# JianCao92/speaker-diarization

Hardware: AMD Instinct MI355X
Metric: diarized audio throughput (CD gw/BIC + CL hi/BIC) (higher is better)
Workload: dtype f64

## Files before the change

include/spkd.h:

```cpp
#ifndef SPKD_H
#define SPKD_H

#include <stddef.h>
#include <stdint.h>

#ifdef __cplusplus
extern "C" {
#endif

#define SPKD_ABI_VERSION 2
#define SPKD_DIM 39
#define SPKD_REC 820

typedef enum {
    SPKD_OK = 0,
    SPKD_EINVAL = 1,
    SPKD_EHIP = 2,
    SPKD_ENONFINITE = 3,
    SPKD_EOVERFLOW = 4,
    SPKD_ENOMEM = 5
} spkd_status;

typedef enum { SPKD_BIC = 0, SPKD_GLR = 1, SPKD_KL2 = 2, SPKD_KL2_PINV = 3 } spkd_kind;

// ... 103 lines not shown
    const int32_t *turn;
    const int64_t *frame_b;
    const int64_t *frame_e;
    const int64_t *index;
    const int64_t *d_index;
    const int64_t *redo_line;
    const int64_t *redo_begin;
    const int64_t *redo_end;
} spkd_gw_lines_view;

spkd_status spkd_gw_batch(spkd_ctx *ctx, const float *d_frames, int64_t n_frames,
                          const int64_t *h_turn_begin, const int64_t *h_turn_end, int64_t n_turns,
                          const spkd_cd_params *params, const int64_t *h_ev_off,
                          const double *h_turn_start_s, const double *h_turn_end_s,
                          const int64_t *h_turn_file_off, const int64_t *h_turn_file_len,
                          double *d_seg_stats, int want_index, spkd_gw_lines_view *view);

int64_t spkd_sw_window_count(int64_t turn_len, double winsize, double winstep);
spkd_status spkd_sw(spkd_ctx *ctx, const float *d_frames, int64_t n_frames,
                    const int64_t *h_turn_begin, const int64_t *h_turn_end, int64_t n_turns,
                    const spkd_cd_params *params, const int64_t *h_d_off, double *h_d);

enum { SPKD_AHC_AUTO = 0, SPKD_AHC_MONO = 1, SPKD_AHC_WIDE = 2 };

typedef struct {
    int32_t variant;
    int32_t kind;
    int32_t max_spk;
    int32_t path;
    double lambdac;
    double threshold;
} spkd_ahc_params;

spkd_status spkd_ahc(spkd_ctx *ctx, const double *d_stats, const int64_t *h_seg_off,
                     int64_t n_problems, const spkd_ahc_params *params,
                     int32_t *h_n_merges, int32_t *h_merge_a, int32_t *h_merge_b,
                     double *h_merge_d, double *h_stat_max, double *h_stat_min);

spkd_status spkd_ahc_matrix(spkd_ctx *ctx, const double *d_stats, int64_t n, const spkd_ahc_params *params,
                            const double *d_matrix, double stat_max_in, double stat_min_in,
                            int32_t *h_n_merges, int32_t *h_merge_a, int32_t *h_merge_b,
                            double *h_merge_d, double *h_stat_max, double *h_stat_min);

spkd_status spkd_ahc_fused(spkd_ctx *ctx, const float *d_frames, int64_t n_frames,
                           const double *d_records, int64_t n_records, int64_t *d_line_index,
                           const int64_t *h_seg_off, int64_t n_problems,
// ... 59 lines not shown
```

speaker-diarization_amd/csrc/spkd_cluster.hpp:

```cpp
#pragma once
#include "spkd_device.hpp"
#include "spkd_quad.hpp"
#include "spkd_tri.hpp"
#include "../../include/spkd.h"

namespace spkd {

constexpr double MAXINT_F = 9223372036854775808.0;
constexpr double PEN_UNIT = 39.0 + 0.5 * 39.0 * 40.0;
constexpr int AUX = 3 * DA;
constexpr int ERR_DEGENERATE_MERGE = 2;

__device__ __forceinline__ unsigned long long dkey(double v) {
    unsigned long long b = (unsigned long long)__double_as_longlong(v);
    return (b >> 63) ? ~b : (b | 0x8000000000000000ull);
}
__device__ __forceinline__ double dkey_inv(unsigned long long k) {
    unsigned long long b = (k >> 63) ? (k & 0x7fffffffffffffffull) : ~k;
    return __longlong_as_double((long long)b);
}
template <bool MAXOP>
__device__ __forceinline__ unsigned wave_red_u32(unsigned x) {
    auto op = [](unsigned a, unsigned b) { return MAXOP ? (a > b ? a : b) : (a < b ? a : b); };
    x = op(x, (unsigned)__builtin_amdgcn_update_dpp((int)x, (int)x, 0xB1, 0xf, 0xf, false));
// ... 476 lines not shown
            }
            if (valid && stat_valid(d)) {
                wmax = (wmax != wmax || d > wmax) ? d : wmax;
                wmin = (wmin != wmin || d < wmin) ? d : wmin;
            }
        }
    }
    if (variant == 1 && (kind == SPKD_KL2 ? lane_id() == 0 : L.t == 0)) {
        if (wmax == wmax) atomicMax(stat_max + p, dkey(wmax));
        if (wmin == wmin) atomicMin(stat_min + p, dkey(wmin));
    }
}

constexpr int AHC_WAVES = 8;
constexpr int AHC_TPB = AHC_WAVES * WAVE;

#ifdef SPKD_PROFILE
__device__ unsigned long long g_step_prof[8];
__device__ unsigned long long g_ahc_prof[8];
#endif
constexpr int NO_COL = 0x7fffffff;
constexpr int AHC_MAX_N = 65536;

__device__ __forceinline__ void refresh_rows(const double* __restrict__ Dm, long long N,
                                             const int32_t* __restrict__ al, int32_t* __restrict__ dirty,
                                             double* __restrict__ rmin, int32_t* __restrict__ rarg,
                                             int32_t* __restrict__ rnan, unsigned long long* masks,
                                             int tid, int wave, int lane) {
    const long long n_chunks = (N + WAVE - 1) / WAVE;
    for (long long ch = wave; ch < n_chunks; ch += AHC_WAVES) {
        const long long rl = ch * WAVE + lane;
        const long long rc = rl < N ? rl : N - 1;
        const int fa = al[rc], fd = dirty[rc];
        const unsigned long long mk = __ballot(rl < N && fa && fd);
        if (lane == 0) masks[ch] = mk;
    }
    __syncthreads();
    int ord = 0;
    for (long long ch = 0; ch < n_chunks; ++ch) {
        const long long r0 = ch * WAVE;
        unsigned long long todo = masks[ch];
        while (todo) {
            const int b = __builtin_ctzll(todo);
            todo &= todo - 1;
            if ((ord++ & (AHC_WAVES - 1)) != wave) continue;
            const long long r = r0 + b;
            const double* row = Dm + r * N;
            double mv = __builtin_huge_val();
            int mc = NO_COL, nc = NO_COL;
            for (long long c0 = 0; c0 < N; c0 += 4 * WAVE) {
                double v[4];
                int a[4];
#pragma unroll
                for (int u = 0; u < 4; ++u) {
                    const long long c = c0 + u * WAVE + lane;
                    const long long cc = c < N ? c : N - 1;
                    a[u] = (c < N) ? al[cc] : 0;
                    v[u] = row[cc];
                }
#pragma unroll
                for (int u = 0; u < 4; ++u) {
                    const int c = (int)(c0 + u * WAVE + lane);
                    if (!a[u]) continue;
                    if (v[u] != v[u]) { if (c < nc) nc = c; continue; }
                    if (v[u] < mv || (v[u] == mv && c < mc)) { mv = v[u]; mc = c; }
                }
            }
            {
                unsigned long long okey;
                unsigned oc;
                wave_argmin_key(mc != NO_COL ? dkey(mv) : ~0ull, (unsigned)mc, okey, oc);
                mv = okey != ~0ull ? dkey_inv(okey) : __builtin_huge_val();
                mc = okey != ~0ull ? (int)oc : NO_COL;
                nc = __any(nc != NO_COL) ? (int)wave_red_u32<false>((unsigned)nc) : NO_COL;
            }
            if (lane == 0) { rmin[r] = mv; rarg[r] = mc; rnan[r] = nc; dirty[r] = 0; }
#ifdef SPKD_PROFILE
            if (lane == 0) atomicAdd(&g_ahc_prof[0], 1ull);
#endif
        }
    }
}

template <bool TWO>
__global__ __launch_bounds__(AHC_TPB) void k_ahc(
        double* __restrict__ ex, double* __restrict__ pk, const int64_t* __restrict__ seg_off,
        int variant, int kind, int max_spk, double lambdac, double threshold,
        double* __restrict__ ld, double* __restrict__ aux,
        double* __restrict__ mat, const int64_t* __restrict__ mat_off,
        int32_t* __restrict__ alive, double* __restrict__ tmp,
        double* __restrict__ rmin_all, int32_t* __restrict__ rcache_all,
        int32_t* __restrict__ out_n, int32_t* __restrict__ out_a, int32_t* __restrict__ out_b,
        double* __restrict__ out_d, unsigned long long* stat_max, unsigned long long* stat_min,
        double* __restrict__ final_max, double* __restrict__ final_min, int* err,
        double* pinv_ws) {
    extern __shared__ int32_t ids[];
    __shared__ double ldsA[QREC];
    __shared__ unsigned long long red3[AHC_WAVES][3];
    __shared__ unsigned long long s_masks[AHC_MAX_N / WAVE];
    __shared__ int s_cnt[2];
    __shared__ int s_nids;
    __shared__ int s_next;
    __shared__ double s_tmax[AHC_WAVES];
    const int tid = threadIdx.x, lane = lane_id(), wave = tid >> 6;
    const QuadLane L = quad_lane();
    const int p = blockIdx.x;
    const int64_t off = seg_off[p];
    const long long N = seg_off[p + 1] - off;
    double* Dm = mat + mat_off[p];
    int32_t* al = alive + off;
    double* ldp = ld + off;
    double* tp = tmp + off;
    double* rmin = rmin_all + off;
    int32_t* rarg = rcache_all + 3 * off;
    int32_t* rnan = rarg + N;
    int32_t* dirty = rnan + N;
    for (long long c = tid; c < N; c += AHC_TPB) { al[c] = 1; dirty[c] = 1; }
    __syncthreads();
    long long m = N;
    int n_merges = 0;
    const long long INF_IDX = 0x7fffffffffffffffLL;
    double fmin = 0.0;
#ifdef SPKD_PROFILE
    unsigned long long ahc_acc[5] = {0ull, 0ull, 0ull, 0ull, 0ull}, ahc_t = clock64();
#define AHC_TICK(i) do { const unsigned long long now_ = clock64(); ahc_acc[i] += now_ - ahc_t; ahc_t = now_; } while (0)
#else
#define AHC_TICK(i) ((void)0)
#endif
    while (true) {
        refresh_rows(Dm, N, al, dirty, rmin, rarg, rnan, s_masks, tid, wave, lane);
        __syncthreads();
        AHC_TICK(0);
        unsigned long long kb = ~0ull, ib = ~0ull, inan = ~0ull;
        for (long long r = tid; r < N; r += AHC_TPB) {
            if (!al[r]) continue;
            const double v = rmin[r];
            const int c = rarg[r], nc = rnan[r];
            if (nc != NO_COL) { const unsigned long long l = (unsigned long long)(r * N + nc); inan = l < inan ? l : inan; }
            if (c != NO_COL) {
                const unsigned long long kv = dkey(v);
                if (kv < kb) { kb = kv; ib = (unsigned long long)(r * N + c); }
            }
        }
        {
            const unsigned long long wk = wave_red_u64<false>(kb);
            const unsigned long long wi = wave_red_u64<false>(kb == wk ? ib : ~0ull);
            const unsigned long long wn = __any(inan != ~0ull) ? wave_red_u64<false>(inan) : ~0ull;
            if (lane == 0) { red3[wave][0] = wk; red3[wave][1] = wi; red3[wave][2] = wn; }
        }
        __syncthreads();
        unsigned long long bk = red3[0][0], bi = red3[0][1], bn = red3[0][2];
#pragma unroll
        for (int w = 1; w < AHC_WAVES; ++w) {
            const unsigned long long ok = red3[w][0], oi = red3[w][1], on = red3[w][2];
            const bool t = ok < bk || (ok == bk && oi < bi);
            bk = t ? ok : bk; bi = t ? oi : bi;
            bn = on < bn ? on : bn;
        }
        const bool has_nan = bn != ~0ull;
        const double mind = has_nan ? __builtin_nan("") : (bi != ~0ull ? dkey_inv(bk) : __builtin_huge_val());
        const long long index = has_nan ? (long long)bn : (bi != ~0ull ? (long long)bi : INF_IDX);
        fmin = mind;
        const bool go = (mind <= threshold) || (max_spk > 0 && m > max_spk);
        if (!go) break;
        AHC_TICK(1);
        const long long r0 = index / N, c0 = index - r0 * N;
        if (r0 == c0) {
            if (tid == 0) atomicOr(err, ERR_DEGENERATE_MERGE);
            break;
        }
        const long long sa = r0 < c0 ? r0 : c0, sb = r0 < c0 ? c0 : r0;
        if (tid < 2) s_cnt[tid] = 0;
        if (tid == 0) { s_nids = 1; s_next = 0; }
        __syncthreads();
        {
            int ca = 0, cb = 0;
            for (long long c = tid; c < sb; c += AHC_TPB) {
                if (al[c]) { cb++; if (c < sa) ca++; }
            }
            ca = __builtin_amdgcn_readlane(wave_scan_i32(ca), WAVE - 1);
            cb = __builtin_amdgcn_readlane(wave_scan_i32(cb), WAVE - 1);
            if (lane == 0 && ca) atomicAdd(&s_cnt[0], ca);
            if (lane == 0 && cb) atomicAdd(&s_cnt[1], cb);
        }
        __syncthreads();
        if (tid == 0) {
            const int64_t o = off + n_merges;
            out_a[o] = s_cnt[0]; out_b[o] = s_cnt[1]; out_d[o] = mind;
            al[sb] = 0;
            ids[0] = (int32_t)sa;
        }
        n_merges++;
        m--;
#ifdef SPKD_PROFILE
        if (tid == 0) atomicAdd(&g_ahc_prof[1], 1ull);
#endif
        double* A = ex + (off + sa) * QREC;
        const double* B = ex + (off + sb) * QREC;
        {
            double* Ap = pk + (off + sa) * REC;
            const double* Bp = pk + (off + sb) * REC;
            constexpr int NQ = (QREC + AHC_TPB - 1) / AHC_TPB, NP = (REC + AHC_TPB - 1) / AHC_TPB;
            double qa[NQ], qb[NQ], pa[NP], pb[NP];
#pragma unroll
            for (int u = 0; u < NQ; ++u) {
                const int e = tid + u * AHC_TPB;
                qa[u] = A[e < QREC ? e : 0]; qb[u] = B[e < QREC ? e : 0];
            }
#pragma unroll
            for (int u = 0; u < NP; ++u) {
                const int e = tid + u * AHC_TPB;
                pa[u] = Ap[e < REC ? e : 0]; pb[u] = Bp[e < REC ? e : 0];
            }
#pragma unroll
            for (int u = 0; u < NQ; ++u) {
                const int e = tid + u * AHC_TPB;
                const double v = qa[u] + qb[u];
                if (e < QREC) { A[e] = v; ldsA[e] = v; }
            }
#pragma unroll
            for (int u = 0; u < NP; ++u) {
                const int e = tid + u * AHC_TPB;
                if (e < REC) Ap[e] = pa[u] + pb[u];
            }
        }
        __syncthreads();
        for (long long c0 = 0; c0 < N; c0 += AHC_TPB) {
            const long long c = c0 + tid;
            const bool take = c < N && c != sa && al[c < N ? c : N - 1];
            const unsigned long long mk = __ballot(take);
            int base = 0;
            if (lane == 0 && mk) base = atomicAdd(&s_nids, __popcll(mk));
            base = __shfl(base, 0);
            if (take) ids[base + __popcll(mk & ((1ull << lane) - 1ull))] = (int32_t)c;
        }
        __syncthreads();
        AHC_TICK(2);
        const int nids = s_nids;
        const double nA = ldsA[QREC_COUNT_AT];
        if (kind == SPKD_KL2) {
            if (wave == 0) {
                double a[DA];
                single_rows_from_qr(A, a);
                const double mean_i = a[D] / nA;
                cov_rows(a, nA);
                kl2_aux_from_cov(a, mean_i, aux + (off + sa) * AUX, pinv_ws);
            }
        } else {
            for (;;) {
                int q4 = 0;
                if (lane == 0) q4 = atomicAdd(&s_next, 1);
                const int base = 4 * __builtin_amdgcn_readfirstlane(q4);
                if (base >= nids) break;
                int k = base + L.m;
                const bool valid = k < nids;
                k = valid ? k : nids - 1;
                const int32_t slot = ids[k];
                const double v = quad_pair_det<TWO>(kind, ldsA, nA, A, ex + (off + slot) * QREC, pk + (off + slot) * REC, k == 0, L, err);
                if (valid && L.t == 0) {
                    if (k == 0) ldp[sa] = log(v); else tp[slot] = v;
                }
            }
        }
        __syncthreads();
        AHC_TICK(3);
        double wmax = __builtin_nan(""), wmin = __builtin_nan("");
        const double ldA = ldp[sa];
        for (long long c = tid; c < N; c += AHC_TPB) {
            if (c == sa || !al[c]) continue;
            double d;
            if (kind == SPKD_KL2) {
                const double* a1 = aux + (off + sa) * AUX;
                const double* a2 = aux + (off + c) * AUX;
                double t1 = 0.0, t2 = 0.0;
                for (int i = 0; i < D; ++i) {
                    const float dm = (float)a1[2 * DA + i] - (float)a2[2 * DA + i];
                    const double delta = (double)dm;
                    t1 += (a1[i] - a2[i]) * (a2[DA + i] - a1[DA + i]);
                    t2 += ((a1[DA + i] + a2[DA + i]) * delta) * delta;
                }
                d = 0.5 * t1 + 0.5 * t2;
            } else {
                const double nC = qr_count(ex + (off + c) * QREC);
                d = finish_distance(kind, lambdac, nA, ldA, nC, ldp[c], log(tp[c]));
            }
            Dm[sa * N + c] = d;
            const int ra = rarg[c], rn = rnan[c];
            if (variant == 1) {
                Dm[c * N + sa] = d;
                if (ra == sa || ra == sb || rn == sa || rn == sb) {
                    if (rn != sa && rn != sb && d < rmin[c]) { rmin[c] = d; rarg[c] = (int)sa; }
                    else dirty[c] = 1;
                }
                else if (d != d) { if ((int)sa < rn) rnan[c] = (int)sa; }
                else if (d < rmin[c] || (d == rmin[c] && (int)sa < ra)) { rmin[c] = d; rarg[c] = (int)sa; }
                if (stat_valid(d)) {
                    wmax = (wmax != wmax || d > wmax) ? d : wmax;
                    wmin = (wmin != wmin || d < wmin) ? d : wmin;
                }
            } else {
                if (ra == sb || rn == sb) dirty[c] = 1;
            }
        }
        if (tid == 0) dirty[sa] = 1;
        if (variant == 1) {
            const unsigned long long kmax = wave_red_u64<true>(wmax == wmax ? dkey(wmax) : 0ull);
            const unsigned long long kmin = wave_red_u64<false>(wmin == wmin ? dkey(wmin) : ~0ull);
            if (lane == 0) {
                if (kmax != 0ull) atomicMax(stat_max + p, kmax);
                if (kmin != ~0ull) atomicMin(stat_min + p, kmin);
            }
        }
        __syncthreads();
        AHC_TICK(4);
    }
#ifdef SPKD_PROFILE
    if (tid == 0) for (int i = 0; i < 5; ++i) atomicAdd(&g_ahc_prof[2 + i], ahc_acc[i]);
#endif
    double tmax = -__builtin_huge_val();
    bool anynan = false;
    for (long long r = wave; r < N; r += AHC_WAVES) {
        if (!al[r]) continue;
        const double* row = Dm + r * N;
        for (long long c = lane; c < N; c += WAVE) {
            if (!al[c]) continue;
            const double v = row[c];
            if (v != v) anynan = true; else tmax = v > tmax ? v : tmax;
        }
    }
#pragma unroll
    for (int s = 1; s < WAVE; s <<= 1) {
        const double t2 = __shfl_xor(tmax, s);
        tmax = t2 > tmax ? t2 : tmax;
    }
    anynan = __any(anynan);
    if (lane == 0) s_tmax[wave] = anynan ? __builtin_nan("") : tmax;
    __syncthreads();
    if (tid == 0) {
        double mx = s_tmax[0];
        for (int w = 1; w < AHC_WAVES; ++w) {
            const double x = s_tmax[w];
            if (mx == mx) mx = (x != x) ? x : (x > mx ? x : mx);
        }
        out_n[p] = n_merges;
        final_max[p] = mx;
        final_min[p] = fmin;
    }
}

__device__ __forceinline__ void ahc_scan_row(const double* __restrict__ row, long long N,
                                             const int32_t* __restrict__ al, bool all_alive,
                                             long long sub_col, double sub_val, int lane,
                                             double& mv, int& mc, int& nc) {
    mv = __builtin_huge_val();
    mc = NO_COL; nc = NO_COL;
    for (long long c0 = 0; c0 < N; c0 += 4 * WAVE) {
        double v[4];
        int a[4];
#pragma unroll
        for (int u = 0; u < 4; ++u) {
            const long long c = c0 + u * WAVE + lane;
            const long long cc = c < N ? c : N - 1;
            a[u] = (c < N) ? (all_alive ? 1 : al[cc]) : 0;
            v[u] = row[cc];
// ... 651 lines not shown
```

speaker-diarization_amd/csrc/spkd_hip.hip:

```cpp
#include <hip/hip_runtime.h>

#include <algorithm>
#include <cmath>
#include <cstdio>
#include <cstdlib>
#include <cstring>
#include <string>
#include <atomic>
#include <thread>
#include <vector>

#include "../../include/spkd.h"
#include "spkd_cd.hpp"
#include "spkd_cluster.hpp"
#include "spkd_device.hpp"
#include "spkd_handoff.hpp"
#include "spkd_stats.hpp"
#include "spkd_mfcc.hpp"
#include "spkd_vad.hpp"

using namespace spkd;

namespace {
constexpr int N_SLOTS = 40;
enum { PIN_GW_TURNS = 0, PIN_GW_LINES, PIN_AHC_OUT, N_PIN };
}

struct spkd_ctx {
    int device = 0;
    hipStream_t stream = nullptr;
    bool own_stream = false;
    bool gw_lds_ok = false;
    int gw_waves = 0;
    unsigned long long init_keys[2] = {0ull, ~0ull};
    int step_waves = 0;
    int step_partners = 0;
    int64_t last_gw_items = 0;
    std::string err;
    int* d_err = nullptr;
    unsigned long long* d_counter = nullptr;
    hipEvent_t ev0 = nullptr, ev1 = nullptr;
    float last_ms = 0.f;
    hipEvent_t ka[SPKD_N_TIMERS] = {}, kb[SPKD_N_TIMERS] = {};
    bool kused[SPKD_N_TIMERS] = {};
    float kms[SPKD_N_TIMERS] = {};
    void* slot[N_SLOTS] = {};
    size_t slot_bytes[N_SLOTS] = {};
    void* pinv_ws = nullptr;
    double* pinv_cur = nullptr;
    void* pin[N_PIN] = {};
    size_t pin_bytes[N_PIN] = {};
    std::vector<int64_t> redo_line, redo_begin, redo_end;
    std::vector<Chunk> redo_chunks;
    std::vector<int64_t> redo_setoff;
    std::vector<int32_t> redo_sets;
};

namespace {

// ... 140 lines not shown
        if (hipStreamCreateWithFlags(&c->stream, hipStreamDefault) != hipSuccess) { delete c; return SPKD_EHIP; }
        c->own_stream = true;
    }
    if (hipMalloc(&c->d_err, sizeof(int)) != hipSuccess ||
        hipMalloc(&c->d_counter, 2 * sizeof(unsigned long long)) != hipSuccess ||
        hipEventCreate(&c->ev0) != hipSuccess || hipEventCreate(&c->ev1) != hipSuccess) {
        spkd_destroy(c);
        return SPKD_EHIP;
    }
    for (int i = 0; i < SPKD_N_TIMERS; ++i)
        if (hipEventCreate(&c->ka[i]) != hipSuccess || hipEventCreate(&c->kb[i]) != hipSuccess) {
            spkd_destroy(c);
            return SPKD_EHIP;
        }
    int lds_max = 0;
    c->gw_lds_ok = hipDeviceGetAttribute(&lds_max, hipDeviceAttributeMaxSharedMemoryPerBlock, device) == hipSuccess &&
                   Gw<4>::LDS_BYTES <= lds_max &&
                   hipFuncSetAttribute((const void*)k_gw<8>, hipFuncAttributeMaxDynamicSharedMemorySize, Gw<8>::LDS_BYTES) == hipSuccess &&
                   hipFuncSetAttribute((const void*)k_gw<4>, hipFuncAttributeMaxDynamicSharedMemorySize, Gw<4>::LDS_BYTES) == hipSuccess &&
                   hipFuncSetAttribute((const void*)k_gw<2>, hipFuncAttributeMaxDynamicSharedMemorySize, Gw<2>::LDS_BYTES) == hipSuccess &&
                   hipFuncSetAttribute((const void*)k_gw<1>, hipFuncAttributeMaxDynamicSharedMemorySize, Gw<1>::LDS_BYTES) == hipSuccess;
    if (const char* e = getenv("SPKD_GW_WAVES")) c->gw_waves = atoi(e);
    if (const char* e = getenv("SPKD_STEP_WAVES")) { const int v = atoi(e); c->step_waves = (v == 4 || v == 8) ? v : 0; }
    if (const char* e = getenv("SPKD_STEP_PARTNERS")) { const int v = atoi(e); c->step_partners = (v == 3 || v == 7 || v == 15) ? v : 0; }
    *out = c;
    return SPKD_OK;
}

spkd_status spkd_create(int device, void* stream, spkd_ctx** out) {
    return create_ctx(device, stream, stream != nullptr, out);
}

spkd_status spkd_create_on_stream(int device, void* stream, spkd_ctx** out) {
    return create_ctx(device, stream, true, out);
}

void spkd_destroy(spkd_ctx* c) {
    if (!c) return;
    (void)hipSetDevice(c->device);
    if (c->stream) (void)hipStreamSynchronize(c->stream);
    for (int i = 0; i < N_SLOTS; ++i)
        if (c->slot[i]) (void)hipFree(c->slot[i]);
    if (c->d_err) (void)hipFree(c->d_err);
    if (c->pinv_ws) (void)hipFree(c->pinv_ws);
    for (int i = 0; i < N_PIN; ++i)
        if (c->pin[i]) (void)hipHostFree(c->pin[i]);
// ... 423 lines not shown
    if (h_stat_max) *h_stat_max = key_to_double(keys[0], true);
    if (h_stat_min) *h_stat_min = key_to_double(keys[1], false);
    return st;
}

namespace {
spkd_status ahc_impl(spkd_ctx* c, const double* d_stats, const int64_t* h_seg_off, int64_t n_prob,
                     const spkd_ahc_params* P, const MatrixPlan& plan, int32_t* h_n_merges, int32_t* h_merge_a,
                     int32_t* h_merge_b, double* h_merge_d, double* h_stat_max, double* h_stat_min) {
    if (!c || !P || n_prob < 0) return SPKD_EINVAL;
    if (n_prob == 0) return SPKD_OK;
    if (!d_stats || !h_seg_off || !h_n_merges || !h_merge_a || !h_merge_b || !h_merge_d ||
        !h_stat_max || !h_stat_min)
        return fail(c, SPKD_EINVAL, "null argument");
    if ((P->variant != 1 && P->variant != 2) || P->kind < 0 || P->kind > 3)
        return fail(c, SPKD_EINVAL, "bad variant / kind");
    for (int64_t p = 0; p < n_prob; ++p)
        if (h_seg_off[p + 1] - h_seg_off[p] < 1) return fail(c, SPKD_EINVAL, "empty clustering problem");
    int64_t n_max = 0;
    for (int64_t p = 0; p < n_prob; ++p) n_max = std::max<int64_t>(n_max, h_seg_off[p + 1] - h_seg_off[p]);
    if (n_max > AHC_MAX_N) return fail(c, SPKD_EINVAL, "clustering problem larger than 65536 records");
    int path = P->path;
    if (path != SPKD_AHC_MONO && path != SPKD_AHC_WIDE) path = n_prob <= 64 ? SPKD_AHC_WIDE : SPKD_AHC_MONO;
    const size_t lds = (size_t)(n_max + 4) * sizeof(int32_t);
    if (path == SPKD_AHC_MONO && lds > 150 * 1024) path = SPKD_AHC_WIDE;
    if (path == SPKD_AHC_WIDE && n_max > STEP_MAX_N)
        return fail(c, SPKD_EINVAL, "clustering problem larger than 16384 records (wide merge loop)");
    AhcBuffers B;
    int64_t n_total = 0;
    std::vector<int64_t> offs;
    std::vector<int32_t> prob_of;
    std::vector<unsigned long long> kmax((size_t)n_prob), kmin((size_t)n_prob);
    std::vector<double> fmax((size_t)n_prob), fmin((size_t)n_prob);
    Call call(c);
    TRY(call.opened);
    spkd_ahc_params Pk = *P;
    TRY(use_kind(c, P->kind, &Pk.kind));
    P = &Pk;
    TRY(ahc_prepare(c, d_stats, h_seg_off, n_prob, P->variant, P->kind, P->lambdac, B, n_total, offs, prob_of, plan));
    void* op = nullptr;
    const size_t out_bytes = (size_t)n_total * (6 * sizeof(int32_t) + 3 * sizeof(double)) +
                             (size_t)n_prob * (sizeof(int32_t) + 2 * sizeof(double)) + 64;
    TRY(scratch(c, S_AHC_OUT, out_bytes, &op));
    double* d_merge_d = (double*)op;
    double* d_tmp = d_merge_d + n_total;
    double* d_rmin = d_tmp + n_total;
    double* d_fmax = d_rmin + n_total;
    double* d_fmin = d_fmax + n_prob;
    int32_t* d_a = (int32_t*)(d_fmin + n_prob);
    int32_t* d_b = d_a + n_total;
    int32_t* d_alive = d_b + n_total;
    int32_t* d_rcache = d_alive + n_total;
    int32_t* d_n = d_rcache + 3 * n_total;
    if (path == SPKD_AHC_MONO) {
        auto kahc = P->kind == SPKD_GLR ? k_ahc<true> : k_ahc<false>;
        if (lds > 48 * 1024)
            (void)hipFuncSetAttribute((const void*)kahc, hipFuncAttributeMaxDynamicSharedMemorySize, (int)lds);
        Timer t(c, SPKD_T_AHC);
        hipLaunchKernelGGL(kahc, dim3((unsigned)n_prob), dim3(AHC_TPB), lds, c->stream,
                           B.ex, B.pk, (const int64_t*)B.seg_off, P->variant, P->kind, P->max_spk, P->lambdac,
                           P->threshold, B.ld, B.aux, B.mat, (const int64_t*)B.mat_off, d_alive, d_tmp,
                           d_rmin, d_rcache, d_n, d_a, d_b, d_merge_d, B.smax, B.smin, d_fmax, d_fmin, c->d_err,
                           c->pinv_cur);
    } else {
        StepArrays Q;
        void *pm = nullptr, *pe = nullptr, *pp = nullptr;
        const size_t nt = (size_t)n_total;
        const size_t misc_bytes = nt * 2 * sizeof(StepSel) + nt * sizeof(double) + nt * sizeof(unsigned long long) +
                                  (size_t)2 * n_prob * sizeof(StepState) + nt * sizeof(int32_t) + 64;
        TRY(scratch(c, S_STEP_MISC, misc_bytes, &pm));
        TRY(scratch(c, S_STEP_EXM, nt * QREC * sizeof(double), &pe));
        TRY(scratch(c, S_STEP_PKM, nt * REC * sizeof(double), &pp));
        Q.ex = B.ex; Q.pk = B.pk; Q.exm = (double*)pe; Q.pkm = (double*)pp;
        Q.sel2 = (StepSel*)pm;
        Q.cnt = (double*)(Q.sel2 + 2 * nt);
        Q.sw = (unsigned long long*)(Q.cnt + nt);
        Q.state2 = (StepState*)(Q.sw + nt);
        Q.death = (int32_t*)(Q.state2 + 2 * n_prob);
        Q.n_total = n_total;
        Q.n_prob = (int32_t)n_prob;
        const int step_waves = c->step_waves ? c->step_waves : (n_max > STEP_WIDE_FROM ? 8 : 4);
        const bool glr_k = P->kind == SPKD_GLR;
        using StepKernel = decltype(&k_ahc_step<false, 4, 3>);
        StepKernel kvar[3];
        if (step_waves == 8) {
// ... 36 lines not shown
                           Q, d_n, d_fmax, d_fmin);
    }
    HIPCHK(c, hipGetLastError());
    HIPCHK(c, hipMemcpyAsync(h_n_merges, d_n, (size_t)n_prob * sizeof(int32_t), hipMemcpyDeviceToHost, c->stream));
    HIPCHK(c, hipMemcpyAsync(h_merge_a, d_a, (size_t)n_total * sizeof(int32_t), hipMemcpyDeviceToHost, c->stream));
    HIPCHK(c, hipMemcpyAsync(h_merge_b, d_b, (size_t)n_total * sizeof(int32_t), hipMemcpyDeviceToHost, c->stream));
    HIPCHK(c, hipMemcpyAsync(h_merge_d, d_merge_d, (size_t)n_total * sizeof(double), hipMemcpyDeviceToHost, c->stream));
    HIPCHK(c, hipMemcpyAsync(kmax.data(), B.smax, (size_t)n_prob * sizeof(unsigned long long), hipMemcpyDeviceToHost, c->stream));
    HIPCHK(c, hipMemcpyAsync(kmin.data(), B.smin, (size_t)n_prob * sizeof(unsigned long long), hipMemcpyDeviceToHost, c->stream));
    HIPCHK(c, hipMemcpyAsync(fmax.data(), d_fmax, (size_t)n_prob * sizeof(double), hipMemcpyDeviceToHost, c->stream));
    HIPCHK(c, hipMemcpyAsync(fmin.data(), d_fmin, (size_t)n_prob * sizeof(double), hipMemcpyDeviceToHost, c->stream));
    const spkd_status st = call.finish();
    for (int64_t p = 0; p < n_prob; ++p) {
        if (P->variant == 1) {
            h_stat_max[p] = key_to_double(kmax[(size_t)p], true);
            h_stat_min[p] = key_to_double(kmin[(size_t)p], false);
        } else {
            h_stat_max[p] = fmax[(size_t)p];
            h_stat_min[p] = fmin[(size_t)p];
        }
    }
    return st;
}
}

spkd_status spkd_ahc(spkd_ctx* c, const double* d_stats, const int64_t* h_seg_off, int64_t n_prob,
                     const spkd_ahc_params* P, int32_t* h_n_merges, int32_t* h_merge_a,
                     int32_t* h_merge_b, double* h_merge_d, double* h_stat_max, double* h_stat_min) {
    return ahc_impl(c, d_stats, h_seg_off, n_prob, P, MatrixPlan(), h_n_merges, h_merge_a, h_merge_b, h_merge_d,
                    h_stat_max, h_stat_min);
}

spkd_status spkd_ahc_matrix(spkd_ctx* c, const double* d_stats, int64_t n, const spkd_ahc_params* P,
                            const double* d_matrix, double stat_max_in, double stat_min_in,
                            int32_t* h_n_merges, int32_t* h_merge_a, int32_t* h_merge_b, double* h_merge_d,
                            double* h_stat_max, double* h_stat_min) {
    if (!c || n < 1) return SPKD_EINVAL;
    if (!d_matrix) return fail(c, SPKD_EINVAL, "ahc_matrix: null matrix");
    const int64_t seg_off[2] = {0, n};
    MatrixPlan plan;
    plan.d_init = d_matrix;
    plan.init_max = stat_max_in;
    plan.init_min = stat_min_in;
    return ahc_impl(c, d_stats, seg_off, 1, P, plan, h_n_merges, h_merge_a, h_merge_b, h_merge_d, h_stat_max, h_stat_min);
}

// ... 827 lines not shown
```

speaker-diarization_amd/hipabi.py:

```python
import ctypes as C
import os

import numpy as np

HERE = os.path.dirname(os.path.abspath(__file__))
LIB_PATH = os.environ.get('SPKD_HIP_LIBRARY') or os.path.join(HERE, 'csrc', 'libspkd_hip.so')

SPKD_OK, SPKD_EINVAL, SPKD_EHIP, SPKD_ENONFINITE, SPKD_EOVERFLOW, SPKD_ENOMEM = range(6)
KINDS = {'BIC': 0, 'GLR': 1, 'KL2': 2, 'KL2P': 3}
WANT_GLR, WANT_KL2, WANT_KL2_PINV = 1, 2, 4
TIMERS = {n: i for i, n in enumerate(['call', 'chunk_stats', 'reduce_sets', 'pair_terms',
                                        'cluster_prep', 'matrix', 'ahc', 'gw', 'sw'])}
REC = 820
DIM = 39

EXPORTS = ['spkd_abi_version', 'spkd_create', 'spkd_create_on_stream', 'spkd_destroy', 'spkd_last_error', 'spkd_sync',
           'spkd_malloc', 'spkd_free', 'spkd_memcpy_h2d', 'spkd_memcpy_d2h', 'spkd_memcpy_d2d',
           'spkd_last_kernel_ms', 'spkd_last_gw_items', 'spkd_set_stats', 'spkd_pair_terms',
           'spkd_distance_matrix', 'spkd_gw_event_capacity', 'spkd_gw_event_capacity_p', 'spkd_gw', 'spkd_gw_ex', 'spkd_gw_fused', 'spkd_gw_batch', 'spkd_ahc_fused', 'spkd_gather_stats', 'spkd_mfcc',
           'spkd_sw_window_count', 'spkd_sw', 'spkd_ahc', 'spkd_ahc_matrix', 'spkd_distance_rows', 'spkd_cluster_in', 'spkd_py2_roundtrip',
           'spkd_labels_from_merges', 'spkd_labels_from_merges_batch', 'spkd_count_flags', 'spkd_gw_lines',
           'spkd_gmm_loglik', 'spkd_vad_viterbi']


class CdParams(C.Structure):
    _fields_ = [('kind', C.c_int32), ('trace', C.c_int32), ('lambdac', C.c_double),
                ('threshold', C.c_double), ('winsize', C.c_double), ('winstep', C.c_double),
                ('deltaws', C.c_double), ('rate', C.c_double)]


class CandLog(C.Structure):
    _fields_ = [('turn', C.c_int32), ('coarse', C.c_int32), ('seq', C.c_int64),
                ('start', C.c_double), ('i', C.c_double), ('d', C.c_double),
                ('n1', C.c_int64), ('n2', C.c_int64)]


class GwLinesView(C.Structure):
    _fields_ = [('n_lines', C.c_int64), ('n_redo', C.c_int64), ('n_win', C.c_void_p), ('times', C.c_void_p),
                ('turn', C.c_void_p), ('frame_b', C.c_void_p), ('frame_e', C.c_void_p), ('index', C.c_void_p),
                ('d_index', C.c_void_p), ('redo_line', C.c_void_p), ('redo_begin', C.c_void_p),
                ('redo_end', C.c_void_p)]


# ... 80 lines not shown
    _check_one_runtime()
    vp, i64, i32, dbl = C.c_void_p, C.c_int64, C.c_int32, C.c_double
    P = C.POINTER
    lib.spkd_abi_version.restype = C.c_int
    lib.spkd_create.argtypes = [C.c_int, vp, P(vp)]
    lib.spkd_create_on_stream.argtypes = [C.c_int, vp, P(vp)]
    lib.spkd_destroy.argtypes = [vp]
    lib.spkd_destroy.restype = None
    lib.spkd_last_error.argtypes = [vp]
    lib.spkd_last_error.restype = C.c_char_p
    lib.spkd_sync.argtypes = [vp]
    lib.spkd_malloc.argtypes = [vp, C.c_size_t, P(vp)]
    lib.spkd_free.argtypes = [vp, vp]
    lib.spkd_memcpy_h2d.argtypes = [vp, vp, vp, C.c_size_t]
    lib.spkd_memcpy_d2h.argtypes = [vp, vp, vp, C.c_size_t]
    lib.spkd_memcpy_d2d.argtypes = [vp, vp, vp, C.c_size_t]
    lib.spkd_last_kernel_ms.argtypes = [vp, C.c_int, P(C.c_float)]
    lib.spkd_last_gw_items.argtypes = [vp, P(C.c_int64)]
    lib.spkd_set_stats.argtypes = [vp, vp, i64, vp, vp, vp, i64, i64, vp]
    lib.spkd_pair_terms.argtypes = [vp, vp, vp, vp, i64, C.c_int, vp]
    lib.spkd_distance_matrix.argtypes = [vp, C.c_int, dbl, vp, i64, vp]
    lib.spkd_gw_event_capacity.argtypes = [i64, dbl]
    lib.spkd_gw_event_capacity.restype = i64
    lib.spkd_gw_event_capacity_p.argtypes = [i64, P(CdParams)]
    lib.spkd_gw_event_capacity_p.restype = i64
    lib.spkd_gw.argtypes = [vp, vp, i64, vp, vp, i64, P(CdParams), vp, vp, vp, vp, vp, vp, vp, vp,
                            vp, i64, P(i64)]
    lib.spkd_gw_ex.argtypes = [vp, vp, i64, vp, vp, i64, P(CdParams), vp, C.c_int, vp, vp, vp, vp, vp, vp,
                               vp, vp, i64, P(i64)]
    lib.spkd_gw_fused.argtypes = [vp, vp, i64, vp, vp, i64, P(CdParams), vp, C.c_int, vp, vp, vp, vp, vp, vp,
                                  vp, vp, vp, i64, P(i64)]
    lib.spkd_gw_batch.argtypes = [vp, vp, i64, vp, vp, i64, P(CdParams), vp, vp, vp, vp, vp, vp, C.c_int, P(GwLinesView)]
    lib.spkd_ahc_fused.argtypes = [vp, vp, i64, vp, i64, vp, vp, i64, vp, vp, vp, i64, P(AhcParams),
                                   P(vp), P(vp), P(vp), P(vp), P(vp)]
    lib.spkd_gather_stats.argtypes = [vp, vp, i64, vp, vp, i64, i64, vp]
    lib.spkd_mfcc.argtypes = [vp, vp, i64, P(MfccParams), vp, vp, vp, vp, vp, vp, P(i64)]
    lib.spkd_sw_window_count.argtypes = [i64, dbl, dbl]
    lib.spkd_sw_window_count.restype = i64
    lib.spkd_sw.argtypes = [vp, vp, i64, vp, vp, i64, P(CdParams), vp, vp]
    lib.spkd_ahc.argtypes = [vp, vp, vp, i64, P(AhcParams), vp, vp, vp, vp, vp, vp]
    lib.spkd_ahc_matrix.argtypes = [vp, vp, i64, P(AhcParams), vp, dbl, dbl, vp, vp, vp, vp, vp, vp]
    lib.spkd_distance_rows.argtypes = [vp, C.c_int, C.c_int, dbl, vp, i64, i64, i64, vp, P(dbl), P(dbl)]
    lib.spkd_cluster_in.argtypes = [vp, vp, i64, C.c_int, dbl, dbl, vp, vp, i64, vp, P(i64), P(i64)]
    lib.spkd_py2_roundtrip.argtypes = [vp, i64]
    lib.spkd_py2_roundtrip.restype = None
    lib.spkd_labels_from_merges.argtypes = [i64, i64, vp, vp, vp]
# ... 427 lines not shown
```

Measured before the change: 1466.

## Keep AHC per-row state and alive bitmask in LDS, restructure merge step

Moves the per-row clustering state (row minima, argmins, NaN columns, dirty flags, log-dets, pair temps, counts) of the monolithic AHC kernel from global memory into LDS when the problem fits, and replaces the alive int array with a shared bitmask. Partner-list construction and merge counts now come from popcounts over the bitmask instead of atomics, cluster counts are cached rather than re-read from stats, and one barrier per iteration is dropped. This removes global-memory traffic and synchronisation in the sequential merge loop, but uses much more LDS per block, which can lower occupancy. A global-state fallback remains available through an environment variable.

```diff
diff --git a/include/spkd.h b/include/spkd.h
--- a/include/spkd.h
+++ b/include/spkd.h
@@ -149,6 +149,8 @@
                     const spkd_cd_params *params, const int64_t *h_d_off, double *h_d);
 
 enum { SPKD_AHC_AUTO = 0, SPKD_AHC_MONO = 1, SPKD_AHC_WIDE = 2 };
+int64_t spkd_ahc_lds_capacity(void);
+int64_t spkd_ahc_lds_bytes(int64_t n_max, int lds_state);
 
 typedef struct {
     int32_t variant;
diff --git a/speaker-diarization_amd/csrc/spkd_cluster.hpp b/speaker-diarization_amd/csrc/spkd_cluster.hpp
--- a/speaker-diarization_amd/csrc/spkd_cluster.hpp
+++ b/speaker-diarization_amd/csrc/spkd_cluster.hpp
@@ -522,17 +522,48 @@
 constexpr int NO_COL = 0x7fffffff;
 constexpr int AHC_MAX_N = 65536;
 
+struct AhcState {
+    double *rmin, *ld, *tmp, *cnt;
+    int32_t *rarg, *rnan, *dirty;
+};
+constexpr size_t AHC_STATE_BYTES = 4 * sizeof(double) + 3 * sizeof(int32_t);
+struct AhcGlobalState {
+    double *rmin, *tmp, *cnt;
+    int32_t* rcache;
+};
+struct AhcShared {
+    double ldsA[QREC];
+    unsigned long long red3[AHC_WAVES][3];
+    unsigned long long masks[AHC_MAX_N / WAVE];
+    unsigned long long alive[AHC_MAX_N / WAVE];
+    double tmax[AHC_WAVES];
+    int next;
+};
+constexpr size_t AHC_LDS_LIMIT = 160 * 1024;
+constexpr size_t ahc_dyn_lds(long long n_max, bool lds_state) {
+    return (lds_state ? (size_t)n_max * AHC_STATE_BYTES : 0) + (size_t)(n_max + 4) * sizeof(int32_t);
+}
+constexpr long long AHC_LDS_CAPACITY =
+    (long long)((AHC_LDS_LIMIT - sizeof(AhcShared) - 4 * sizeof(int32_t)) / (AHC_STATE_BYTES + sizeof(int32_t)));
+static_assert(sizeof(AhcShared) + ahc_dyn_lds(AHC_LDS_CAPACITY, true) <= AHC_LDS_LIMIT &&
+              sizeof(AhcShared) + ahc_dyn_lds(AHC_LDS_CAPACITY + 1, true) > AHC_LDS_LIMIT, "LDS capacity of k_ahc");
+
+__device__ __forceinline__ bool ahc_alive(const unsigned long long* alive, long long c) {
+    return (alive[c >> 6] >> (c & 63)) & 1ull;
+}
+__device__ __forceinline__ unsigned long long bits_below(long long k) {
+    return k <= 0 ? 0ull : (k >= 64 ? ~0ull : (1ull << k) - 1ull);
+}
+
 __device__ __forceinline__ void refresh_rows(const double* __restrict__ Dm, long long N,
-                                             const int32_t* __restrict__ al, int32_t* __restrict__ dirty,
-                                             double* __restrict__ rmin, int32_t* __restrict__ rarg,
-                                             int32_t* __restrict__ rnan, unsigned long long* masks,
-                                             int tid, int wave, int lane) {
+                                             const unsigned long long* alive, const AhcState& S,
+                                             unsigned long long* masks, int tid, int wave, int lane) {
     const long long n_chunks = (N + WAVE - 1) / WAVE;
     for (long long ch = wave; ch < n_chunks; ch += AHC_WAVES) {
         const long long rl = ch * WAVE + lane;
         const long long rc = rl < N ? rl : N - 1;
-        const int fa = al[rc], fd = dirty[rc];
-        const unsigned long long mk = __ballot(rl < N && fa && fd);
+        const int fd = S.dirty[rc];
+        const unsigned long long mk = __ballot(rl < N && fd) & alive[ch];
         if (lane == 0) masks[ch] = mk;
     }
     __syncthreads();
@@ -555,7 +586,7 @@
                 for (int u = 0; u < 4; ++u) {
                     const long long c = c0 + u * WAVE + lane;
                     const long long cc = c < N ? c : N - 1;
-                    a[u] = (c < N) ? al[cc] : 0;
+                    a[u] = (c < N) & (int)((alive[cc >> 6] >> (cc & 63)) & 1ull);
                     v[u] = row[cc];
                 }
 #pragma unroll
@@ -574,7 +605,7 @@
                 mc = okey != ~0ull ? (int)oc : NO_COL;
                 nc = __any(nc != NO_COL) ? (int)wave_red_u32<false>((unsigned)nc) : NO_COL;
             }
-            if (lane == 0) { rmin[r] = mv; rarg[r] = mc; rnan[r] = nc; dirty[r] = 0; }
+            if (lane == 0) { S.rmin[r] = mv; S.rarg[r] = mc; S.rnan[r] = nc; S.dirty[r] = 0; }
 #ifdef SPKD_PROFILE
             if (lane == 0) atomicAdd(&g_ahc_prof[0], 1ull);
 #endif
@@ -582,40 +613,42 @@
     }
 }
 
-template <bool TWO>
+template <bool TWO, bool LDS_STATE>
 __global__ __launch_bounds__(AHC_TPB) void k_ahc(
         double* __restrict__ ex, double* __restrict__ pk, const int64_t* __restrict__ seg_off,
         int variant, int kind, int max_spk, double lambdac, double threshold,
         double* __restrict__ ld, double* __restrict__ aux,
-        double* __restrict__ mat, const int64_t* __restrict__ mat_off,
-        int32_t* __restrict__ alive, double* __restrict__ tmp,
-        double* __restrict__ rmin_all, int32_t* __restrict__ rcache_all,
+        double* __restrict__ mat, const int64_t* __restrict__ mat_off, AhcGlobalState G,
         int32_t* __restrict__ out_n, int32_t* __restrict__ out_a, int32_t* __restrict__ out_b,
         double* __restrict__ out_d, unsigned long long* stat_max, unsigned long long* stat_min,
         double* __restrict__ final_max, double* __restrict__ final_min, int* err,
         double* pinv_ws) {
-    extern __shared__ int32_t ids[];
-    __shared__ double ldsA[QREC];
-    __shared__ unsigned long long red3[AHC_WAVES][3];
-    __shared__ unsigned long long s_masks[AHC_MAX_N / WAVE];
-    __shared__ int s_cnt[2];
-    __shared__ int s_nids;
-    __shared__ int s_next;
-    __shared__ double s_tmax[AHC_WAVES];
+    extern __shared__ double ahc_dyn[];
+    __shared__ AhcShared sh;
     const int tid = threadIdx.x, lane = lane_id(), wave = tid >> 6;
     const QuadLane L = quad_lane();
     const int p = blockIdx.x;
     const int64_t off = seg_off[p];
     const long long N = seg_off[p + 1] - off;
+    const long long n_chunks = (N + WAVE - 1) / WAVE;
     double* Dm = mat + mat_off[p];
-    int32_t* al = alive + off;
-    double* ldp = ld + off;
-    double* tp = tmp + off;
-    double* rmin = rmin_all + off;
-    int32_t* rarg = rcache_all + 3 * off;
-    int32_t* rnan = rarg + N;
-    int32_t* dirty = rnan + N;
-    for (long long c = tid; c < N; c += AHC_TPB) { al[c] = 1; dirty[c] = 1; }
+    AhcState S;
+    int32_t* ids;
+    if constexpr (LDS_STATE) {
+        S.rmin = ahc_dyn; S.ld = S.rmin + N; S.tmp = S.ld + N; S.cnt = S.tmp + N;
+        S.rarg = (int32_t*)(S.cnt + N); S.rnan = S.rarg + N; S.dirty = S.rnan + N;
+        ids = S.dirty + N;
+    } else {
+        S.rmin = G.rmin + off; S.ld = ld + off; S.tmp = G.tmp + off; S.cnt = G.cnt + off;
+        S.rarg = G.rcache + 3 * off; S.rnan = S.rarg + N; S.dirty = S.rnan + N;
+        ids = (int32_t*)ahc_dyn;
+    }
+    for (long long c = tid; c < N; c += AHC_TPB) {
+        S.dirty[c] = 1;
+        S.cnt[c] = qr_count(ex + (off + c) * QREC);
+        if constexpr (LDS_STATE) S.ld[c] = ld[off + c];
+    }
+    for (long long ch = tid; ch < n_chunks; ch += AHC_TPB) sh.alive[ch] = bits_below(N - ch * WAVE);
     __syncthreads();
     long long m = N;
     int n_merges = 0;
@@ -628,14 +661,14 @@
 #define AHC_TICK(i) ((void)0)
 #endif
     while (true) {
-        refresh_rows(Dm, N, al, dirty, rmin, rarg, rnan, s_masks, tid, wave, lane);
+        refresh_rows(Dm, N, sh.alive, S, sh.masks, tid, wave, lane);
         __syncthreads();
         AHC_TICK(0);
         unsigned long long kb = ~0ull, ib = ~0ull, inan = ~0ull;
         for (long long r = tid; r < N; r += AHC_TPB) {
-            if (!al[r]) continue;
-            const double v = rmin[r];
-            const int c = rarg[r], nc = rnan[r];
+            if (!ahc_alive(sh.alive, r)) continue;
+            const double v = S.rmin[r];
+            const int c = S.rarg[r], nc = S.rnan[r];
             if (nc != NO_COL) { const unsigned long long l = (unsigned long long)(r * N + nc); inan = l < inan ? l : inan; }
             if (c != NO_COL) {
                 const unsigned long long kv = dkey(v);
@@ -646,13 +679,13 @@
             const unsigned long long wk = wave_red_u64<false>(kb);
             const unsigned long long wi = wave_red_u64<false>(kb == wk ? ib : ~0ull);
             const unsigned long long wn = __any(inan != ~0ull) ? wave_red_u64<false>(inan) : ~0ull;
-            if (lane == 0) { red3[wave][0] = wk; red3[wave][1] = wi; red3[wave][2] = wn; }
+            if (lane == 0) { sh.red3[wave][0] = wk; sh.red3[wave][1] = wi; sh.red3[wave][2] = wn; }
         }
         __syncthreads();
-        unsigned long long bk = red3[0][0], bi = red3[0][1], bn = red3[0][2];
+        unsigned long long bk = sh.red3[0][0], bi = sh.red3[0][1], bn = sh.red3[0][2];
 #pragma unroll
         for (int w = 1; w < AHC_WAVES; ++w) {
-            const unsigned long long ok = red3[w][0], oi = red3[w][1], on = red3[w][2];
+            const unsigned long long ok = sh.red3[w][0], oi = sh.red3[w][1], on = sh.red3[w][2];
             const bool t = ok < bk || (ok == bk && oi < bi);
             bk = t ? ok : bk; bi = t ? oi : bi;
             bn = on < bn ? on : bn;
@@ -670,74 +703,73 @@
             break;
         }
         const long long sa = r0 < c0 ? r0 : c0, sb = r0 < c0 ? c0 : r0;
-        if (tid < 2) s_cnt[tid] = 0;
-        if (tid == 0) { s_nids = 1; s_next = 0; }
-        __syncthreads();
-        {
+        double* A = ex + (off + sa) * QREC;
+        const double* B = ex + (off + sb) * QREC;
+        double* Ap = pk + (off + sa) * REC;
+        const double* Bp = pk + (off + sb) * REC;
+        constexpr int NQ = (QREC + AHC_TPB - 1) / AHC_TPB, NP = (REC + AHC_TPB - 1) / AHC_TPB;
+        double qa[NQ], qb[NQ], pa[NP], pb[NP];
+#pragma unroll
+        for (int u = 0; u < NQ; ++u) {
+            const int e = tid + u * AHC_TPB;
+            qa[u] = A[e < QREC ? e : 0]; qb[u] = B[e < QREC ? e : 0];
+        }
+#pragma unroll
+        for (int u = 0; u < NP; ++u) {
+            const int e = tid + u * AHC_TPB;
+            pa[u] = Ap[e < REC ? e : 0]; pb[u] = Bp[e < REC ? e : 0];
+        }
+        if (wave == 0) {
             int ca = 0, cb = 0;
-            for (long long c = tid; c < sb; c += AHC_TPB) {
-                if (al[c]) { cb++; if (c < sa) ca++; }
+            for (long long j = lane; j * WAVE < sb; j += WAVE) {
+                const unsigned long long w = sh.alive[j];
+                ca += __popcll(w & bits_below(sa - j * WAVE));
+                cb += __popcll(w & bits_below(sb - j * WAVE));
             }
             ca = __builtin_amdgcn_readlane(wave_scan_i32(ca), WAVE - 1);
             cb = __builtin_amdgcn_readlane(wave_scan_i32(cb), WAVE - 1);
-            if (lane == 0 && ca) atomicAdd(&s_cnt[0], ca);
-            if (lane == 0 && cb) atomicAdd(&s_cnt[1], cb);
-        }
-        __syncthreads();
-        if (tid == 0) {
-            const int64_t o = off + n_merges;
-            out_a[o] = s_cnt[0]; out_b[o] = s_cnt[1]; out_d[o] = mind;
-            al[sb] = 0;
-            ids[0] = (int32_t)sa;
-        }
+            if (lane == 0) {
+                const int64_t o = off + n_merges;
+                out_a[o] = ca; out_b[o] = cb; out_d[o] = mind;
+                S.cnt[sa] += S.cnt[sb];
+                ids[0] = (int32_t)sa;
+                sh.next = 0;
+            }
+        }
+        auto partners = [&](long long j) {
+            unsigned long long w = sh.alive[j];
+            if (j == (sa >> 6)) w &= ~(1ull << (sa & 63));
+            if (j == (sb >> 6)) w &= ~(1ull << (sb & 63));
+            return w;
+        };
+        for (long long ch = wave; ch < n_chunks; ch += AHC_WAVES) {
+            int pre = 0;
+            for (long long j = lane; j < ch; j += WAVE) pre += __popcll(partners(j));
+            pre = __builtin_amdgcn_readlane(wave_scan_i32(pre), WAVE - 1);
+            const unsigned long long mk = partners(ch);
+            if ((mk >> lane) & 1ull) ids[1 + pre + __popcll(mk & ((1ull << lane) - 1ull))] = (int32_t)(ch * WAVE + lane);
+        }
+        if (tid == 0) sh.alive[sb >> 6] &= ~(1ull << (sb & 63));
         n_merges++;
         m--;
 #ifdef SPKD_PROFILE
         if (tid == 0) atomicAdd(&g_ahc_prof[1], 1ull);
 #endif
-        double* A = ex + (off + sa) * QREC;
-        const double* B = ex + (off + sb) * QREC;
-        {
-            double* Ap = pk + (off + sa) * REC;
-            const double* Bp = pk + (off + sb) * REC;
-            constexpr int NQ = (QREC + AHC_TPB - 1) / AHC_TPB, NP = (REC + AHC_TPB - 1) / AHC_TPB;
-            double qa[NQ], qb[NQ], pa[NP], pb[NP];
-#pragma unroll
-            for (int u = 0; u < NQ; ++u) {
-                const int e = tid + u * AHC_TPB;
-                qa[u] = A[e < QREC ? e : 0]; qb[u] = B[e < QREC ? e : 0];
-            }
-#pragma unroll
-            for (int u = 0; u < NP; ++u) {
-                const int e = tid + u * AHC_TPB;
-                pa[u] = Ap[e < REC ? e : 0]; pb[u] = Bp[e < REC ? e : 0];
-            }
-#pragma unroll
-            for (int u = 0; u < NQ; ++u) {
-                const int e = tid + u * AHC_TPB;
-                const double v = qa[u] + qb[u];
-                if (e < QREC) { A[e] = v; ldsA[e] = v; }
-            }
-#pragma unroll
-            for (int u = 0; u < NP; ++u) {
-                const int e = tid + u * AHC_TPB;
-                if (e < REC) Ap[e] = pa[u] + pb[u];
-            }
-        }
-        __syncthreads();
-        for (long long c0 = 0; c0 < N; c0 += AHC_TPB) {
-            const long long c = c0 + tid;
-            const bool take = c < N && c != sa && al[c < N ? c : N - 1];
-            const unsigned long long mk = __ballot(take);
-            int base = 0;
-            if (lane == 0 && mk) base = atomicAdd(&s_nids, __popcll(mk));
-            base = __shfl(base, 0);
-            if (take) ids[base + __popcll(mk & ((1ull << lane) - 1ull))] = (int32_t)c;
+#pragma unroll
+        for (int u = 0; u < NQ; ++u) {
+            const int e = tid + u * AHC_TPB;
+            const double v = qa[u] + qb[u];
+            if (e < QREC) { A[e] = v; sh.ldsA[e] = v; }
+        }
+#pragma unroll
+        for (int u = 0; u < NP; ++u) {
+            const int e = tid + u * AHC_TPB;
+            if (e < REC) Ap[e] = pa[u] + pb[u];
         }
         __syncthreads();
         AHC_TICK(2);
-        const int nids = s_nids;
-        const double nA = ldsA[QREC_COUNT_AT];
+        const int nids = (int)m;
+        const double nA = sh.ldsA[QREC_COUNT_AT];
         if (kind == SPKD_KL2) {
             if (wave == 0) {
                 double a[DA];
@@ -749,25 +781,26 @@
         } else {
             for (;;) {
                 int q4 = 0;
-                if (lane == 0) q4 = atomicAdd(&s_next, 1);
+                if (lane == 0) q4 = atomicAdd(&sh.next, 1);
                 const int base = 4 * __builtin_amdgcn_readfirstlane(q4);
                 if (base >= nids) break;
                 int k = base + L.m;
                 const bool valid = k < nids;
                 k = valid ? k : nids - 1;
                 const int32_t slot = ids[k];
-                const double v = quad_pair_det<TWO>(kind, ldsA, nA, A, ex + (off + slot) * QREC, pk + (off + slot) * REC, k == 0, L, err);
+                const double v = quad_pair_det<TWO>(kind, sh.ldsA, nA, A, ex + (off + slot) * QREC, pk + (off + slot) * REC, k == 0, L, err);
                 if (valid && L.t == 0) {
-                    if (k == 0) ldp[sa] = log(v); else tp[slot] = v;
+                    if (k == 0) S.ld[sa] = log(v); else S.tmp[slot] = v;
                 }
             }
         }
         __syncthreads();
         AHC_TICK(3);
         double wmax = __builtin_nan(""), wmin = __builtin_nan("");
-        const double ldA = ldp[sa];
+        const double ldA = S.ld[sa];
         for (long long c = tid; c < N; c += AHC_TPB) {
-            if (c == sa || !al[c]) continue;
+            if (c == sa) { S.dirty[c] = 1; continue; }
+            if (!ahc_alive(sh.alive, c)) continue;
             double d;
             if (kind == SPKD_KL2) {
                 const double* a1 = aux + (off + sa) * AUX;
@@ -781,28 +814,26 @@
                 }
                 d = 0.5 * t1 + 0.5 * t2;
             } else {
-                const double nC = qr_count(ex + (off + c) * QREC);
-                d = finish_distance(kind, lambdac, nA, ldA, nC, ldp[c], log(tp[c]));
+                d = finish_distance(kind, lambdac, nA, ldA, S.cnt[c], S.ld[c], log(S.tmp[c]));
             }
             Dm[sa * N + c] = d;
-            const int ra = rarg[c], rn = rnan[c];
+            const int ra = S.rarg[c], rn = S.rnan[c];
             if (variant == 1) {
                 Dm[c * N + sa] = d;
                 if (ra == sa || ra == sb || rn == sa || rn == sb) {
-                    if (rn != sa && rn != sb && d < rmin[c]) { rmin[c] = d; rarg[c] = (int)sa; }
-                    else dirty[c] = 1;
+                    if (rn != sa && rn != sb && d < S.rmin[c]) { S.rmin[c] = d; S.rarg[c] = (int)sa; }
+                    else S.dirty[c] = 1;
                 }
-                else if (d != d) { if ((int)sa < rn) rnan[c] = (int)sa; }
-                else if (d < rmin[c] || (d == rmin[c] && (int)sa < ra)) { rmin[c] = d; rarg[c] = (int)sa; }
+                else if (d != d) { if ((int)sa < rn) S.rnan[c] = (int)sa; }
+                else if (d < S.rmin[c] || (d == S.rmin[c] && (int)sa < ra)) { S.rmin[c] = d; S.rarg[c] = (int)sa; }
                 if (stat_valid(d)) {
                     wmax = (wmax != wmax || d > wmax) ? d : wmax;
                     wmin = (wmin != wmin || d < wmin) ? d : wmin;
                 }
             } else {
-                if (ra == sb || rn == sb) dirty[c] = 1;
-            }
-        }
-        if (tid == 0) dirty[sa] = 1;
+                if (ra == sb || rn == sb) S.dirty[c] = 1;
+            }
+        }
         if (variant == 1) {
             const unsigned long long kmax = wave_red_u64<true>(wmax == wmax ? dkey(wmax) : 0ull);
             const unsigned long long kmin = wave_red_u64<false>(wmin == wmin ? dkey(wmin) : ~0ull);
@@ -811,7 +842,6 @@
                 if (kmin != ~0ull) atomicMin(stat_min + p, kmin);
             }
         }
-        __syncthreads();
         AHC_TICK(4);
     }
 #ifdef SPKD_PROFILE
@@ -820,10 +850,10 @@
     double tmax = -__builtin_huge_val();
     bool anynan = false;
     for (long long r = wave; r < N; r += AHC_WAVES) {
-        if (!al[r]) continue;
+        if (!ahc_alive(sh.alive, r)) continue;
         const double* row = Dm + r * N;
         for (long long c = lane; c < N; c += WAVE) {
-            if (!al[c]) continue;
+            if (!ahc_alive(sh.alive, c)) continue;
             const double v = row[c];
             if (v != v) anynan = true; else tmax = v > tmax ? v : tmax;
         }
@@ -834,12 +864,12 @@
         tmax = t2 > tmax ? t2 : tmax;
     }
     anynan = __any(anynan);
-    if (lane == 0) s_tmax[wave] = anynan ? __builtin_nan("") : tmax;
+    if (lane == 0) sh.tmax[wave] = anynan ? __builtin_nan("") : tmax;
     __syncthreads();
     if (tid == 0) {
-        double mx = s_tmax[0];
+        double mx = sh.tmax[0];
         for (int w = 1; w < AHC_WAVES; ++w) {
-            const double x = s_tmax[w];
+            const double x = sh.tmax[w];
             if (mx == mx) mx = (x != x) ? x : (x > mx ? x : mx);
         }
         out_n[p] = n_merges;
diff --git a/speaker-diarization_amd/csrc/spkd_hip.hip b/speaker-diarization_amd/csrc/spkd_hip.hip
--- a/speaker-diarization_amd/csrc/spkd_hip.hip
+++ b/speaker-diarization_amd/csrc/spkd_hip.hip
@@ -35,6 +35,7 @@
     unsigned long long init_keys[2] = {0ull, ~0ull};
     int step_waves = 0;
     int step_partners = 0;
+    bool ahc_global_state = false;
     int64_t last_gw_items = 0;
     std::string err;
     int* d_err = nullptr;
@@ -221,6 +222,7 @@
                    hipFuncSetAttribute((const void*)k_gw<1>, hipFuncAttributeMaxDynamicSharedMemorySize, Gw<1>::LDS_BYTES) == hipSuccess;
     if (const char* e = getenv("SPKD_GW_WAVES")) c->gw_waves = atoi(e);
     if (const char* e = getenv("SPKD_STEP_WAVES")) { const int v = atoi(e); c->step_waves = (v == 4 || v == 8) ? v : 0; }
+    if (const char* e = getenv("SPKD_AHC_STATE")) c->ahc_global_state = std::string(e) == "global";
     if (const char* e = getenv("SPKD_STEP_PARTNERS")) { const int v = atoi(e); c->step_partners = (v == 3 || v == 7 || v == 15) ? v : 0; }
     *out = c;
     return SPKD_OK;
@@ -690,7 +692,8 @@
     if (n_max > AHC_MAX_N) return fail(c, SPKD_EINVAL, "clustering problem larger than 65536 records");
     int path = P->path;
     if (path != SPKD_AHC_MONO && path != SPKD_AHC_WIDE) path = n_prob <= 64 ? SPKD_AHC_WIDE : SPKD_AHC_MONO;
-    const size_t lds = (size_t)(n_max + 4) * sizeof(int32_t);
+    const bool lds_state = n_max <= AHC_LDS_CAPACITY && !c->ahc_global_state;
+    const size_t lds = ahc_dyn_lds(n_max, lds_state);
     if (path == SPKD_AHC_MONO && lds > 150 * 1024) path = SPKD_AHC_WIDE;
     if (path == SPKD_AHC_WIDE && n_max > STEP_MAX_N)
         return fail(c, SPKD_EINVAL, "clustering problem larger than 16384 records (wide merge loop)");
@@ -706,29 +709,36 @@
     TRY(use_kind(c, P->kind, &Pk.kind));
     P = &Pk;
     TRY(ahc_prepare(c, d_stats, h_seg_off, n_prob, P->variant, P->kind, P->lambdac, B, n_total, offs, prob_of, plan));
+    const bool global_state = path == SPKD_AHC_MONO && !lds_state;
     void* op = nullptr;
-    const size_t out_bytes = (size_t)n_total * (6 * sizeof(int32_t) + 3 * sizeof(double)) +
+    const size_t out_bytes = (size_t)n_total * (2 * sizeof(int32_t) + sizeof(double)) +
+                             (global_state ? (size_t)n_total * (3 * sizeof(int32_t) + 3 * sizeof(double)) : 0) +
                              (size_t)n_prob * (sizeof(int32_t) + 2 * sizeof(double)) + 64;
     TRY(scratch(c, S_AHC_OUT, out_bytes, &op));
     double* d_merge_d = (double*)op;
-    double* d_tmp = d_merge_d + n_total;
-    double* d_rmin = d_tmp + n_total;
-    double* d_fmax = d_rmin + n_total;
+    double* d_fmax = d_merge_d + n_total;
     double* d_fmin = d_fmax + n_prob;
-    int32_t* d_a = (int32_t*)(d_fmin + n_prob);
+    AhcGlobalState G = {nullptr, nullptr, nullptr, nullptr};
+    double* d_end = d_fmin + n_prob;
+    if (global_state) {
+        G.rmin = d_end; G.tmp = G.rmin + n_total; G.cnt = G.tmp + n_total;
+        d_end = G.cnt + n_total;
+    }
+    int32_t* d_a = (int32_t*)d_end;
     int32_t* d_b = d_a + n_total;
-    int32_t* d_alive = d_b + n_total;
-    int32_t* d_rcache = d_alive + n_total;
-    int32_t* d_n = d_rcache + 3 * n_total;
+    int32_t* d_n = d_b + n_total;
+    if (global_state) G.rcache = d_n + n_prob;
     if (path == SPKD_AHC_MONO) {
-        auto kahc = P->kind == SPKD_GLR ? k_ahc<true> : k_ahc<false>;
-        if (lds > 48 * 1024)
+        const bool two = P->kind == SPKD_GLR;
+        auto kahc = lds_state ? (two ? k_ahc<true, true> : k_ahc<false, true>)
+                              : (two ? k_ahc<true, false> : k_ahc<false, false>);
+        if (sizeof(AhcShared) + lds > 48 * 1024)
             (void)hipFuncSetAttribute((const void*)kahc, hipFuncAttributeMaxDynamicSharedMemorySize, (int)lds);
         Timer t(c, SPKD_T_AHC);
         hipLaunchKernelGGL(kahc, dim3((unsigned)n_prob), dim3(AHC_TPB), lds, c->stream,
                            B.ex, B.pk, (const int64_t*)B.seg_off, P->variant, P->kind, P->max_spk, P->lambdac,
-                           P->threshold, B.ld, B.aux, B.mat, (const int64_t*)B.mat_off, d_alive, d_tmp,
-                           d_rmin, d_rcache, d_n, d_a, d_b, d_merge_d, B.smax, B.smin, d_fmax, d_fmin, c->d_err,
+                           P->threshold, B.ld, B.aux, B.mat, (const int64_t*)B.mat_off, G,
+                           d_n, d_a, d_b, d_merge_d, B.smax, B.smin, d_fmax, d_fmin, c->d_err,
                            c->pinv_cur);
     } else {
         StepArrays Q;
@@ -811,6 +821,12 @@
     }
     return st;
 }
+}
+
+int64_t spkd_ahc_lds_capacity(void) { return AHC_LDS_CAPACITY; }
+
+int64_t spkd_ahc_lds_bytes(int64_t n_max, int lds_state) {
+    return n_max < 0 ? -1 : (int64_t)(sizeof(AhcShared) + ahc_dyn_lds(n_max, lds_state != 0));
 }
 
 spkd_status spkd_ahc(spkd_ctx* c, const double* d_stats, const int64_t* h_seg_off, int64_t n_prob,
diff --git a/speaker-diarization_amd/hipabi.py b/speaker-diarization_amd/hipabi.py
--- a/speaker-diarization_amd/hipabi.py
+++ b/speaker-diarization_amd/hipabi.py
@@ -18,7 +18,7 @@
            'spkd_malloc', 'spkd_free', 'spkd_memcpy_h2d', 'spkd_memcpy_d2h', 'spkd_memcpy_d2d',
            'spkd_last_kernel_ms', 'spkd_last_gw_items', 'spkd_set_stats', 'spkd_pair_terms',
            'spkd_distance_matrix', 'spkd_gw_event_capacity', 'spkd_gw_event_capacity_p', 'spkd_gw', 'spkd_gw_ex', 'spkd_gw_fused', 'spkd_gw_batch', 'spkd_ahc_fused', 'spkd_gather_stats', 'spkd_mfcc',
-           'spkd_sw_window_count', 'spkd_sw', 'spkd_ahc', 'spkd_ahc_matrix', 'spkd_distance_rows', 'spkd_cluster_in', 'spkd_py2_roundtrip',
+           'spkd_sw_window_count', 'spkd_sw', 'spkd_ahc', 'spkd_ahc_lds_capacity', 'spkd_ahc_lds_bytes', 'spkd_ahc_matrix', 'spkd_distance_rows', 'spkd_cluster_in', 'spkd_py2_roundtrip',
            'spkd_labels_from_merges', 'spkd_labels_from_merges_batch', 'spkd_count_flags', 'spkd_gw_lines',
            'spkd_gmm_loglik', 'spkd_vad_viterbi']
 
@@ -145,6 +145,10 @@
     lib.spkd_distance_matrix.argtypes = [vp, C.c_int, dbl, vp, i64, vp]
     lib.spkd_gw_event_capacity.argtypes = [i64, dbl]
     lib.spkd_gw_event_capacity.restype = i64
+    lib.spkd_ahc_lds_capacity.argtypes = []
+    lib.spkd_ahc_lds_capacity.restype = i64
+    lib.spkd_ahc_lds_bytes.argtypes = [i64, C.c_int]
+    lib.spkd_ahc_lds_bytes.restype = i64
     lib.spkd_gw_event_capacity_p.argtypes = [i64, P(CdParams)]
     lib.spkd_gw_event_capacity_p.restype = i64
     lib.spkd_gw.argtypes = [vp, vp, i64, vp, vp, i64, P(CdParams), vp, vp, vp, vp, vp, vp, vp, vp,
```

Result: no change. 1478, median of 6 (+0.8%).
